# ml-rust/splintr

Measured on AMD Instinct MI355X. Metric: encode_batch MB/s (bytes in), higher is better.
Workload: dtype u8

## Files before the change

### splintr_amd/csrc/spl_common.h

```cpp
#pragma once
#include <stdint.h>

#if defined(__HIPCC__)
#include <hip/hip_runtime.h>
#define SPL_HD __host__ __device__ __forceinline__
#else
#define SPL_HD inline
#endif

namespace spl {

enum : uint32_t {
    C_P = 0,
    C_AP = 1,
    C_SP = 2,
    C_WS = 3,
    C_NL = 4,
    C_N = 5,
    C_LU = 6, C_LL = 7, C_LT = 8, C_LM = 9, C_LO = 10,
    C_M = 11,
    C_EOT = 12,
    C_WEND = 13,
    C_CONT = 15
};
#define SPL_BIT(c) (1u << (c))
constexpr uint32_t M_L = SPL_BIT(C_LU) | SPL_BIT(C_LL) | SPL_BIT(C_LT) | SPL_BIT(C_LM) | SPL_BIT(C_LO);
constexpr uint32_t M_S = SPL_BIT(C_SP) | SPL_BIT(C_WS) | SPL_BIT(C_NL);
constexpr uint32_t M_OTHER = SPL_BIT(C_P) | SPL_BIT(C_AP) | SPL_BIT(C_M);
constexpr uint32_t M_X = SPL_BIT(C_P) | SPL_BIT(C_AP) | SPL_BIT(C_SP) | SPL_BIT(C_WS) | SPL_BIT(C_M);
constexpr uint32_t M_U = SPL_BIT(C_LU) | SPL_BIT(C_LT) | SPL_BIT(C_LM) | SPL_BIT(C_LO) | SPL_BIT(C_M);
constexpr uint32_t M_W = SPL_BIT(C_LL) | SPL_BIT(C_LM) | SPL_BIT(C_LO) | SPL_BIT(C_M);
constexpr uint32_t M_UW = SPL_BIT(C_LM) | SPL_BIT(C_LO) | SPL_BIT(C_M);

constexpr uint32_t CB_CLASS = 0x0F, CB_SYNC = 0x10, CB_TSTART = 0x20, CB_LEN_SHIFT = 6;

enum : int { PAT_CL100K = 0, PAT_O200K = 1, PAT_MISTRAL_V3 = 2 };

struct alignas(16) Quad { uint32_t x, y, z, w; };
struct ShortEnt {
    uint32_t k0, k1, k2;
    uint32_t id_len;
};
constexpr int SPL_SHORT_BUCKET = 4;
constexpr int SPL_TINY_WORDS = 2;
constexpr int SPL_TINY_MAX = 4;
constexpr int SPL_T8_WORDS = 3;
constexpr int SPL_T8_MAX = 8;
constexpr int SPL_TINY_SALT_BITS = 16, SPL_T8_SALT_BITS = 10, SPL_F4_MASK_BITS = 6;
struct LongEnt {
    uint32_t tag;
    uint32_t id;
    uint32_t off;
    uint32_t len;
};
constexpr uint32_t SPL_EMPTY = 0xFFFFFFFFu;
constexpr int SPL_SHORT_MAX = 12;
constexpr uint64_t SPL_PAIR_EMPTY = ~0ull;
constexpr int SPL_PAIR_BUCKET = 4;
constexpr uint32_t SPL_ID_BITS = 21;
constexpr uint32_t SPL_ID_MASK = (1u << SPL_ID_BITS) - 1;
constexpr uint32_t SPL_NO_RANK = 0xFFFFFFFFu;
constexpr uint32_t SPL_OVF_BIT = 1u << 23;

struct P8Bucket { uint32_t a, b; };
struct alignas(8) PfxEnt { uint32_t lm, id2; };

struct alignas(64) MemoEnt {
    uint32_t key[8];
    uint32_t meta0;
    uint32_t meta1;
    uint32_t ids[6];
};
static_assert(sizeof(MemoEnt) == 64, "one cache line");
struct alignas(64) MemoExt {
    uint32_t ids[8];
    uint32_t ends[2];
    uint32_t pad[6];
};
static_assert(sizeof(MemoExt) == 64, "one cache line");
struct alignas(32) MemoHi { uint32_t k[8]; };
constexpr int SPL_MEMO_MAX_LEN = 32, SPL_MEMO_MAX_LEN2 = 64, SPL_MEMO_TOK1 = 6, SPL_MEMO_MAX_TOK = 14;
constexpr uint32_t SPL_MEMO_LOG_WORDS = 12;
constexpr uint32_t SPL_MEMO_LOG_WORDS2 = 20;
constexpr uint32_t SPL_MEMO_LOG_REGIONS = 64;

struct DeviceTables {
    const uint16_t* ucls_stage1;
    const uint8_t* ucls_stage2;
    uint32_t ucls_shift;
    uint32_t cjk_fast;
    const ShortEnt* short_tab; uint32_t short_mask;
    const uint32_t* tiny_tab;  uint32_t tiny_mask;
    const uint32_t* t8_tab;    uint32_t t8_mask;
    const LongEnt* long_tab;   uint32_t long_mask;
    const uint8_t* key_blob;
    const uint64_t* pair_tab;  uint32_t pair_mask;
    const uint32_t* byte_id;
    uint32_t max_key_len;
    uint32_t pattern;
    uint32_t all_bytes;
    uint32_t id_limit;
    const P8Bucket* p8_tab;    uint32_t p8_mask;
    const uint16_t* len_mask;  uint32_t tiny_free, t8_free;
    uint32_t ascii_base;
    const uint32_t* akind;
    const PfxEnt* pfx;
    const uint16_t* filt4;    uint32_t filt4_shift;
    const MemoEnt* memo;      uint32_t memo_mask;
    const MemoExt* memo_ext;
    const MemoEnt* memo2;     uint32_t memo2_mask;
    const MemoExt* memo2_ext; const MemoHi* memo2_hi;
};
SPL_HD uint32_t hash_f4(uint32_t w0) { return w0 * 0x9E3779B1u; }

SPL_HD uint32_t mix32(uint32_t h) {
    h ^= h >> 16; h *= 0x7feb352du; h ^= h >> 15; h *= 0x846ca68bu; h ^= h >> 16;
    return h;
}
SPL_HD uint32_t hash_t8(uint32_t k0, uint32_t k1, uint32_t len, uint32_t salt = 0) {
    return mix32(k0 * 0x9E3779B1u ^ (k1 * 0x85EBCA77u + 0x165667B1u) ^ (len * 0x27D4EB2Fu) ^ (salt * 0xC2B2AE3Du));
}
SPL_HD uint32_t hash_tiny(uint32_t k0, uint32_t len, uint32_t salt = 0) { return hash_t8(k0, 0u, len, salt); }
SPL_HD uint32_t hash_p8(uint32_t k0, uint32_t k1) { return hash_t8(k0, k1, 9u); }
SPL_HD uint32_t p8_tag(uint32_t k0, uint32_t k1) {
    return mix32(k0 * 0x85EBCA77u ^ (k1 * 0xC2B2AE3Du + 0x27D4EB2Fu)) % 0xFFFFFEu + 1u;
}
SPL_HD uint32_t p8_match(uint32_t e0, uint32_t e1, uint32_t tag) {
    const uint32_t t0 = e0 >> 8, t1 = e1 >> 8;
    uint32_t l = 0;
    if (e0 != 0 && (t0 == tag || t0 == 0xFFFFFFu)) l = e0 & 0xFFu;
    if (e1 != 0 && (t1 == tag || t1 == 0xFFFFFFu) && (e1 & 0xFFu) > l) l = e1 & 0xFFu;
    return l;
}
SPL_HD uint32_t hash_short(uint32_t k0, uint32_t k1, uint32_t k2, uint32_t len, uint32_t salt = 0) {
    uint32_t h = k0 * 0x9E3779B1u ^ (k1 * 0x85EBCA77u + 0x165667B1u) ^ (k2 * 0xC2B2AE3Du) ^ (len * 0x27D4EB2Fu) ^ (salt * 0x165667B1u);
    return mix32(h);
}
SPL_HD uint32_t hash_long_step(uint32_t h, uint32_t w) { h = (h ^ w) * 0x9E3779B1u; return (h << 13) | (h >> 19); }
SPL_HD uint32_t hash_long_fin(uint32_t h, uint32_t len) { return mix32(h ^ len); }
SPL_HD uint32_t hash_long_tag(uint32_t h) { return mix32(h * 0x85EBCA77u + 0x3C6EF372u); }
template <int KW> SPL_HD uint32_t hash_memo_w(const uint32_t (&k)[KW], uint32_t n) {
    uint32_t h = n * 0x27D4EB2Fu + 0x165667B1u;
    for (int i = 0; i < KW; i++) { h = (h ^ k[i]) * 0x9E3779B1u; h = (h << 13) | (h >> 19); }
    return mix32(h);
}
SPL_HD uint32_t hash_memo(const uint32_t (&k)[8], uint32_t n) { return hash_memo_w<8>(k, n); }
SPL_HD uint32_t memo_slot2(uint32_t h, uint32_t mask) { const uint32_t g = ((h >> 17) | (h << 15)) * 0x85EBCA77u; return ((g ^ (g >> 15)) & mask) ^ 1u; }
SPL_HD uint32_t hash_pair(uint32_t l, uint32_t r) { return mix32(l * 0x9E3779B1u + r * 0x85EBCA77u + 0x27D4EB2Fu); }
SPL_HD uint64_t pair_key(uint32_t l, uint32_t r) { return (uint64_t)l | ((uint64_t)r << SPL_ID_BITS); }
constexpr uint64_t SPL_PAIR_KEY_MASK = (1ull << (2 * SPL_ID_BITS)) - 1;

}
```

### splintr_amd/csrc/spl_k_memo.h

```cpp
#pragma once

namespace spl {


__device__ __forceinline__ uint32_t memo_meta0(uint32_t n, uint32_t t) { return 0x80000000u | (t << 8) | n; }
constexpr uint32_t MEMO_SEEDED = 0x40000000u;
constexpr uint32_t MEMO_SEED_KEEP_IDS = 32768u;

constexpr uint32_t MISS_KNOWN = 0x80000000u;
#define MISS_N(item) (((item) >> 16) & 0x7FFFu)

#ifndef SPL_MEMO_SKIP_C
#define SPL_MEMO_SKIP_C 1
#endif
template <bool LONG, class TX, class Emit>
__device__ __forceinline__ int memo_probe(const DeviceTables& T, const TX& tx, int p, int n, Emit emit) {
    constexpr int KW = LONG ? 16 : 8;
    uint32_t k[KW];
#pragma unroll
    for (int i = 0; i < KW; i++) k[i] = 4 * i < n ? mask_tail(tx.load32(p + 4 * i), n - 4 * i) : 0u;
    const uint32_t h = hash_memo_w<KW>(k, (uint32_t)n);
    const MemoEnt* const tab = LONG ? T.memo2 : T.memo;
    const MemoExt* const ext = LONG ? T.memo2_ext : T.memo_ext;
    const uint32_t mask = LONG ? T.memo2_mask : T.memo_mask;
    const uint32_t nf = (uint32_t)(LONG ? n - SPL_MEMO_MAX_LEN : n);
    uint32_t slot = h & mask;
#pragma nounroll
    for (int way = 0; way < 2; way++) {
        const Quad* q = reinterpret_cast<const Quad*>(tab + slot);
        const Quad a = q[0], c = (SPL_MEMO_SKIP_C && n <= 16) ? Quad{0u, 0u, 0u, 0u} : q[1], m = q[2], d = q[3];
        bool eq = (a.x == k[0]) & (a.y == k[1]) & (a.z == k[2]) & (a.w == k[3]) & (c.x == k[4]) & (c.y == k[5]) & (c.z == k[6]) & (c.w == k[7]) &
                  ((m.x & 0x8000003Fu) == (0x80000000u | nf));
        if (LONG && eq) {
            const Quad* hq = reinterpret_cast<const Quad*>(T.memo2_hi + slot);
            const Quad h0 = hq[0], h1 = hq[1];
            eq = (h0.x == k[KW - 8]) & (h0.y == k[KW - 7]) & (h0.z == k[KW - 6]) & (h0.w == k[KW - 5]) &
                 (h1.x == k[KW - 4]) & (h1.y == k[KW - 3]) & (h1.z == k[KW - 2]) & (h1.w == k[KW - 1]);
        }
        if (eq) {
            const uint32_t nt = (m.x >> 8) & 15u;
            if (nt == 0u) return 2;
            const uint32_t ids[6] = {m.z, m.w, d.x, d.y, d.z, d.w};
            int at = 0;
#pragma unroll
            for (int t = 0; t < SPL_MEMO_TOK1; t++)
                if ((uint32_t)t < nt) { emit(p + at, ids[t]); if (t < 5) at = (int)((m.y >> (6 * t)) & 63u); }
            if (nt > (uint32_t)SPL_MEMO_TOK1) {
                const Quad* x = reinterpret_cast<const Quad*>(ext + slot);
                const Quad e0 = x[0], e1 = x[1], e2 = x[2];
                const uint32_t xi[8] = {e0.x, e0.y, e0.z, e0.w, e1.x, e1.y, e1.z, e1.w};
#pragma unroll
                for (int t = 0; t < 8; t++)
                    if ((uint32_t)(t + SPL_MEMO_TOK1) < nt) {
                        at = (int)(((t < 5 ? e2.x : e2.y) >> (6 * (t % 5))) & 63u);
                        emit(p + at, xi[t]);
                    }
            }
            return 1;
        }
        if (!(m.x >> 31)) return 0;
        slot = memo_slot2(h, mask);
    }
    return 0;
}

template <bool LONG, class TX>
__device__ __forceinline__ void memo_log_part(const Batch& b, const TX& tx, const uint32_t* list, uint32_t m16, uint32_t c16, uint32_t m64, uint32_t tile) {
    constexpr int KW = LONG ? 16 : 8;
    constexpr uint32_t LW = LONG ? SPL_MEMO_LOG_WORDS2 : SPL_MEMO_LOG_WORDS;
    const uint32_t lane = tidx() & 63u;
    auto eligible = [&](uint32_t item) {
        const uint32_t n = MISS_N(item);
        return !(item & MISS_KNOWN) && (LONG ? n > (uint32_t)SPL_MEMO_MAX_LEN && n <= (uint32_t)SPL_MEMO_MAX_LEN2 : n <= (uint32_t)SPL_MEMO_MAX_LEN);
    };
    uint32_t n_el = 0;
    if (!LONG) for (uint32_t i0 = 0; i0 < m16; i0 += 64u) n_el += (uint32_t)__popcll(__ballot(i0 + lane < m16 && eligible(list[i0 + lane])));
    for (uint32_t i0 = 0; i0 < m64; i0 += 64u) n_el += (uint32_t)__popcll(__ballot(i0 + lane < m64 && eligible(list[c16 + i0 + lane])));
    if (!n_el) return;
    const uint32_t cap = LONG ? b.mlog2_cap : b.mlog_cap;
    const uint32_t region = tile % SPL_MEMO_LOG_REGIONS;
    uint32_t base = 0;
    if (lane == 0u) base = atomicAdd(&b.mlog_cnt[(LONG ? SPL_MEMO_LOG_REGIONS : 0) + region], n_el);
    base = (uint32_t)__builtin_amdgcn_readfirstlane((int)base);
    if (base >= cap) return;
    const uint32_t ask = cap / 2u < 512u ? cap / 2u : 512u;
    if (lane == 0u && base < ask && base + n_el >= ask) *b.mflag = 1u;
    uint32_t* const out = (LONG ? b.mlog2 : b.mlog) + ((size_t)region * cap) * LW;
    auto put = [&](uint32_t slot, uint32_t item) {
        if (base + slot >= cap) return;
        const int p = (int)(item & 0xFFFFu), n = (int)MISS_N(item);
        uint32_t* e = out + (size_t)(base + slot) * LW;
        e[0] = (uint32_t)n;
#pragma unroll
        for (int i = 0; i < KW; i++) e[1 + i] = 4 * i < n ? mask_tail(tx.load32(p + 4 * i), n - 4 * i) : 0u;
    };
    uint32_t slot = 0;
    for (int part = LONG ? 1 : 0; part < 2; part++) {
        const uint32_t cnt = part ? m64 : m16, at = part ? c16 : 0u;
        for (uint32_t i0 = 0; i0 < cnt; i0 += 64u) {
            const uint32_t i = i0 + lane;
            const uint32_t item = i < cnt ? list[at + i] : MISS_KNOWN;
            const bool el = i < cnt && eligible(item);
            const unsigned long long em = __ballot(el);
            if (el) put(slot + mbcnt64(em), item);
            slot += (uint32_t)__popcll(em);
        }
    }
}
template <class TX>
__device__ __forceinline__ void memo_log(const Batch& b, const TX& tx, const uint32_t* list, uint32_t m16, uint32_t c16, uint32_t m64, uint32_t tile) {
    memo_log_part<false>(b, tx, list, m16, c16, m64, tile);
    if (b.mlog2 && m64) memo_log_part<true>(b, tx, list, m16, c16, m64, tile);
}

constexpr int MEMO_FILL_NT = 128, MEMO_FILL_NT2 = 64;
template <int NT_> struct MemoNodes {
    uint32_t* id_; uint32_t* rk_;
    __device__ __forceinline__ uint32_t& id(int i) { return id_[i * NT_]; }
    __device__ __forceinline__ uint32_t& rk(int i) { return rk_[i * NT_]; }
};
struct MemoKeyAcc {
    const uint32_t* k;
    __device__ __forceinline__ uint32_t txt(int q) const { return (k[q >> 2] >> (8 * (q & 3))) & 0xFFu; }
};
template <bool LONG>
__global__ __launch_bounds__(LONG ? MEMO_FILL_NT2 : MEMO_FILL_NT) void k_memo_fill(DeviceTables T, MemoEnt* memo, MemoExt* memo_ext, MemoHi* memo_hi, const uint32_t* mlog,
                                                                               const uint32_t* mlog_cnt, uint32_t mlog_cap, uint32_t* claim, uint32_t round, unsigned long long* stats) {
    constexpr int KW = LONG ? 16 : 8, NTF = LONG ? MEMO_FILL_NT2 : MEMO_FILL_NT, NMAX = LONG ? SPL_MEMO_MAX_LEN2 : SPL_MEMO_MAX_LEN;
    constexpr uint32_t LW = LONG ? SPL_MEMO_LOG_WORDS2 : SPL_MEMO_LOG_WORDS;
    const uint32_t region = blockIdx.y, i = blockIdx.x * blockDim.x + threadIdx.x;
    const uint32_t cnt = mlog_cnt[region] < mlog_cap ? mlog_cnt[region] : mlog_cap;
    if (i >= cnt) return;
    const uint32_t* e = mlog + ((size_t)region * mlog_cap + i) * LW;
    const uint32_t n = e[0];
    uint32_t k[KW];
#pragma unroll
    for (int w = 0; w < KW; w++) k[w] = e[1 + w];
    if (n < (LONG ? (uint32_t)SPL_MEMO_MAX_LEN + 1u : 2u) || n > (uint32_t)NMAX) return;
    const uint32_t mask = LONG ? T.memo2_mask : T.memo_mask;
    const uint32_t nf = LONG ? n - (uint32_t)SPL_MEMO_MAX_LEN : n;
    const uint32_t h = hash_memo_w<KW>(k, n);
    const uint32_t slots[2] = {h & mask, memo_slot2(h, mask)};
    auto holds = [&](uint32_t sl) {
        const MemoEnt* me = memo + sl;
        bool same = (me->meta0 & 0x8000003Fu) == (0x80000000u | nf);
#pragma unroll
        for (int w = 0; w < 8; w++) same = same && me->key[w] == k[w];
        if (LONG) {
#pragma unroll
            for (int w = 0; w < 8; w++) same = same && memo_hi[sl].k[w] == k[KW - 8 + w];
        }
        return same;
    };
    const bool taken0 = (memo[slots[0]].meta0 >> 31) != 0u, taken1 = (memo[slots[1]].meta0 >> 31) != 0u;
    if ((taken0 && holds(slots[0])) || (taken0 && taken1 && holds(slots[1]))) return;
    MemoEnt* me = nullptr;
    if (!taken0) { if (atomicExch(&claim[slots[0]], round) != round) me = memo + slots[0]; }
    if (!me && taken0 && !taken1) { if (atomicExch(&claim[slots[1]], round) != round) me = memo + slots[1]; }
    if (!me && taken0 && taken1) {
        const bool spare_seed = (!(round & 1u) || memo[slots[0]].ids[0] < MEMO_SEED_KEEP_IDS) && (memo[slots[0]].meta0 & MEMO_SEEDED) && !(memo[slots[1]].meta0 & MEMO_SEEDED);
        const uint32_t ev = slots[spare_seed ? 1 : 0];
        if (atomicExch(&claim[ev], round) != round) me = memo + ev;
    }
    if (!me) return;
    __shared__ uint32_t s_id[NMAX * NTF], s_rk[NMAX * NTF];
    MemoNodes<NTF> s{s_id + threadIdx.x, s_rk + threadIdx.x};
    const MemoKeyAcc tx{k};
    bpe_serial(T, s, tx, 0, (int)n);
    uint32_t ids[SPL_MEMO_MAX_TOK], ends = 0, ends2[2] = {0u, 0u}, nt = 0;
#pragma unroll
    for (int t = 0; t < SPL_MEMO_MAX_TOK; t++) ids[t] = 0u;
    bool fits = true;
    for (uint32_t q = 0; q < n; q++) {
        const uint32_t id = s.id((int)q);
        if (id == SPL_DEAD) continue;
        if (nt >= 1u && nt <= 5u) ends |= q << (6u * (nt - 1u));
        else if (nt >= 6u && nt <= 13u) ends2[(nt - 6u) / 5u] |= q << (6u * ((nt - 6u) % 5u));
        if (id >= T.id_limit || nt >= (uint32_t)SPL_MEMO_MAX_TOK) { fits = false; break; }
        ids[nt++] = id;
    }
    me->meta0 = 0u;
#pragma unroll
    for (int w = 0; w < 8; w++) me->key[w] = k[w];
    if (LONG) {
        MemoHi* const mh = memo_hi + (me - memo);
// ... 38 lines not shown
```

### splintr_amd/csrc/spl_k_merge.h

```cpp
#pragma once

namespace spl {

struct LdsAcc {
    const uint8_t* rec_;
    const uint8_t* txt_;
    __device__ __forceinline__ uint32_t rec(int q) const { return rec_[q]; }
    __device__ __forceinline__ uint32_t txt(int q) const { return txt_[q]; }
    __device__ __forceinline__ uint32_t load32(int p) const {
        const uint32_t* w = reinterpret_cast<const uint32_t*>(txt_) + (p >> 2);
        return __builtin_amdgcn_alignbyte(w[1], w[0], p & 3);
    }
};

extern "C" __device__ int spl_writelane(int src, int lane, int old) __asm("llvm.amdgcn.writelane.i32");
#define write_lane(v, s, lane_) spl_writelane((int)(s), (lane_), (v))

struct WaveBV {
    uint32_t x;
    __device__ __forceinline__ WaveBV operator&(const WaveBV& o) const { return WaveBV{x & o.x}; }
    __device__ __forceinline__ WaveBV operator|(const WaveBV& o) const { return WaveBV{x | o.x}; }
    __device__ __forceinline__ WaveBV operator~() const { return WaveBV{~x}; }
    __device__ __forceinline__ WaveBV shl1() const {
        const uint32_t prev = (uint32_t)__builtin_amdgcn_update_dpp(0, (int)x, 0x138, 0xF, 0xF, true);
        return WaveBV{(x << 1) | (prev >> 31)};
    }
    __device__ __forceinline__ WaveBV shr1() const {
        const uint32_t next = (uint32_t)__builtin_amdgcn_update_dpp(0, (int)x, 0x130, 0xF, 0xF, true);
        return WaveBV{(x >> 1) | (next << 31)};
    }
    __device__ __forceinline__ bool any() const { return __any(x != 0u); }
};

struct MaskLdsAcc {
    const uint8_t* rec_;
    const uint8_t* txt_;
    const uint32_t* mk_;
    int nbw_, w_;
    bool eot_;
    __device__ __forceinline__ uint32_t rec(int q) const { return rec_[q]; }
    __device__ __forceinline__ uint32_t txt(int q) const { return txt_[q]; }
    __device__ __forceinline__ uint32_t mw(int which, int w) const { return mk_[which * nbw_ + w]; }
    __device__ __forceinline__ int wbits() const { return w_; }
    __device__ __forceinline__ bool end_is_eot() const { return eot_; }
};

constexpr int LONG_SMALL_NMAX = 128;
__device__ __forceinline__ void push_long(const Batch& b, uint32_t pos, uint32_t len) {
    if (len <= (uint32_t)LONG_SMALL_NMAX) {
        const uint32_t i = atomicAdd(&b.qcount[2], 1u);
        if (i < b.qcaplong) b.qlong[i] = make_uint2(pos, len);
    } else {
        const uint32_t i = atomicAdd(&b.qcount[4], 1u);
        if (i < b.qcaplong) b.qlong[b.qcaplong - 1u - i] = make_uint2(pos, len);
    }
}

__device__ __forceinline__ uint32_t row16_min(uint32_t x) {
#ifndef SPL_NO_DPP_ASM
    asm volatile("s_nop 1\n\tv_min_u32_dpp %0, %0, %0 quad_perm:[1,0,3,2] row_mask:0xf bank_mask:0xf\n\t"
                 "s_nop 1\n\tv_min_u32_dpp %0, %0, %0 quad_perm:[2,3,0,1] row_mask:0xf bank_mask:0xf\n\t"
                 "s_nop 1\n\tv_min_u32_dpp %0, %0, %0 row_half_mirror row_mask:0xf bank_mask:0xf\n\t"
                 "s_nop 1\n\tv_min_u32_dpp %0, %0, %0 row_mirror row_mask:0xf bank_mask:0xf"
                 : "+v"(x));
    return x;
#else
    auto step = [](uint32_t v, uint32_t y) { return y < v ? y : v; };
    x = step(x, (uint32_t)__builtin_amdgcn_update_dpp((int)x, (int)x, 0xB1, 0xF, 0xF, false));
    x = step(x, (uint32_t)__builtin_amdgcn_update_dpp((int)x, (int)x, 0x4E, 0xF, 0xF, false));
    x = step(x, (uint32_t)__builtin_amdgcn_update_dpp((int)x, (int)x, 0x141, 0xF, 0xF, false));
    x = step(x, (uint32_t)__builtin_amdgcn_update_dpp((int)x, (int)x, 0x140, 0xF, 0xF, false));
    return x;
#endif
}
#ifndef SPL_PAIR_SHORT
#define SPL_PAIR_SHORT 1
#endif
__device__ __forceinline__ uint32_t row_min_sub(uint32_t x, bool whole_row) {
    asm volatile("s_nop 1\n\tv_min_u32_dpp %0, %0, %0 quad_perm:[1,0,3,2] row_mask:0xf bank_mask:0xf\n\t"
                 "s_nop 1\n\tv_min_u32_dpp %0, %0, %0 quad_perm:[2,3,0,1] row_mask:0xf bank_mask:0xf\n\t"
                 "s_nop 1\n\tv_min_u32_dpp %0, %0, %0 row_half_mirror row_mask:0xf bank_mask:0xf"
                 : "+v"(x));
    uint32_t y = x;
    asm volatile("s_nop 1\n\tv_min_u32_dpp %0, %0, %0 row_mirror row_mask:0xf bank_mask:0xf" : "+v"(y));
    return whole_row ? y : x;
}
template <int GW> __device__ __forceinline__ uint32_t group_min(uint32_t x, int sub = GW) {
    if (GW == 16 && SPL_PAIR_SHORT) return row_min_sub(x, sub == 16);
    x = row16_min(x);
    if (GW == 32) {
#ifndef SPL_NO_PERMLANE_SWAP
        const auto r = __builtin_amdgcn_permlane16_swap(x, x, false, false);
        const uint32_t a = r[0], c = r[1];
        x = a < c ? a : c;
#else
        const uint32_t y = (uint32_t)__builtin_amdgcn_ds_swizzle((int)x, 0x401F);
        x = y < x ? y : x;
#endif
    }
    return x;
}

__device__ __forceinline__ uint32_t wave_scan_incl(uint32_t x) {
    x += (uint32_t)__builtin_amdgcn_update_dpp(0, (int)x, 0x111, 0xF, 0xF, true);
    x += (uint32_t)__builtin_amdgcn_update_dpp(0, (int)x, 0x112, 0xF, 0xF, true);
    x += (uint32_t)__builtin_amdgcn_update_dpp(0, (int)x, 0x114, 0xF, 0xF, true);
    x += (uint32_t)__builtin_amdgcn_update_dpp(0, (int)x, 0x118, 0xF, 0xF, true);
    x += (uint32_t)__builtin_amdgcn_update_dpp(0, (int)x, 0x142, 0xA, 0xF, false);
    x += (uint32_t)__builtin_amdgcn_update_dpp(0, (int)x, 0x143, 0xC, 0xF, false);
    return x;
}

__device__ __forceinline__ uint32_t wave_scan_max(uint32_t x) {
    auto mx = [](uint32_t a, int b) { return a > (uint32_t)b ? a : (uint32_t)b; };
    x = mx(x, __builtin_amdgcn_update_dpp(0, (int)x, 0x111, 0xF, 0xF, true));
    x = mx(x, __builtin_amdgcn_update_dpp(0, (int)x, 0x112, 0xF, 0xF, true));
    x = mx(x, __builtin_amdgcn_update_dpp(0, (int)x, 0x114, 0xF, 0xF, true));
    x = mx(x, __builtin_amdgcn_update_dpp(0, (int)x, 0x118, 0xF, 0xF, true));
    x = mx(x, __builtin_amdgcn_update_dpp(0, (int)x, 0x142, 0xA, 0xF, false));
    x = mx(x, __builtin_amdgcn_update_dpp(0, (int)x, 0x143, 0xC, 0xF, false));
    return x;
}

__device__ __forceinline__ uint32_t nib_transpose8(uint32_t v) {
    const uint32_t l = tidx() & 7u;
    {
        uint32_t t = (uint32_t)__builtin_amdgcn_update_dpp((int)v, (int)v, 0x104, 0xF, 0x5, false);
        t = (uint32_t)__builtin_amdgcn_update_dpp((int)t, (int)v, 0x114, 0xF, 0xA, false);
        const uint32_t km = (l & 4u) ? 0xFFFF0000u : 0x0000FFFFu;
        const uint32_t y = __builtin_amdgcn_alignbit(t, t, 16);
        v = (v & km) | (y & ~km);
    }
    {
        const uint32_t t = (uint32_t)__builtin_amdgcn_update_dpp((int)v, (int)v, 0x4E, 0xF, 0xF, false);
        const uint32_t km = (l & 2u) ? 0xFF00FF00u : 0x00FF00FFu;
        const uint32_t y = __builtin_amdgcn_alignbit(t, t, (l & 2u) ? 8u : 24u);
        v = (v & km) | (y & ~km);
    }
    {
        const uint32_t t = (uint32_t)__builtin_amdgcn_update_dpp((int)v, (int)v, 0xB1, 0xF, 0xF, false);
        const uint32_t km = (l & 1u) ? 0xF0F0F0F0u : 0x0F0F0F0Fu;
        const uint32_t y = __builtin_amdgcn_alignbit(t, t, (l & 1u) ? 4u : 28u);
        v = (v & km) | (y & ~km);
    }
    return v;
}

template <int NW> __device__ __forceinline__ int next_set_bit(const uint32_t (&a)[NW], int from) {
    int res = -1;
#pragma unroll
    for (int w = NW - 1; w >= 0; w--) {
        uint32_t x = a[w];
        const int lo = from - 32 * w;
        if (lo >= 32) x = 0;
        else if (lo > 0) x &= ~((1u << lo) - 1u);
        if (x) res = 32 * w + __ffs((int)x) - 1;
    }
    return res;
}
template <int NW> __device__ __forceinline__ int prev_set_bit(const uint32_t (&a)[NW], int before) {
    int res = -1;
#pragma unroll
    for (int w = 0; w < NW; w++) {
        uint32_t x = a[w];
        const int hi = before - 32 * w;
// ... 1024 lines not shown
```

### splintr_amd/csrc/spl_k_pretok.h

```cpp
#pragma once

namespace spl {

#ifndef SPL_XCD_MAP
#define SPL_XCD_MAP 1
#endif
__device__ __forceinline__ uint32_t xcd_tile() {
    if (!SPL_XCD_MAP) return blockIdx.x;
    const uint32_t x = blockIdx.x & 7u, j = blockIdx.x >> 3, q = gridDim.x >> 3, r = gridDim.x & 7u;
    return x * q + (x < r ? x : r) + j;
}
constexpr uint32_t PRETOK_E_TSTART = 1u, PRETOK_E_SKIP = 2u, PRETOK_E_GAPS = 4u, PRETOK_E_EXT = 8u, PRETOK_E_FUSE = 64u, PRETOK_E_MEMO1 = 128u;
inline uint32_t pretok_flags(const DeviceTables& T, const Batch& b) {
    return (b.tstart ? PRETOK_E_TSTART : 0u) | (b.skip ? PRETOK_E_SKIP : 0u) | (b.ext_gaps ? PRETOK_E_GAPS : 0u) |
           (b.ext_starts ? PRETOK_E_EXT : 0u) | (T.pattern << 4) | (b.ftc ? PRETOK_E_FUSE : 0u) | ((b.memo_first && T.memo) ? PRETOK_E_MEMO1 : 0u) |
           (b.tile0 << 8);
}
struct PretokKernargs {
    const uint8_t* e_text; const uint64_t* e_doc_off; uint32_t e_n_bytes, e_n_docs; unsigned long long* e_dbg;
    const uint32_t* e_akind; uint32_t e_flags; DeviceTables T; Batch b;
};
#define PRETOK_EARLY(T, b) (b).text, (b).doc_off, (b).n_bytes, (b).n_docs, (b).dbg, (T).akind, pretok_flags(T, b)
template <int TB_, int RH_>
__global__ __launch_bounds__(NT) __attribute__((amdgpu_waves_per_eu(SPL_PRETOK_WAVES)))
// ... 338 lines not shown
                } else if (KPAT != PAT_CL100K) {
                    const bool mistral = KPAT == PAT_MISTRAL_V3;
                    const O200kStartMasks<WaveBV> om{WaveBV{ld(MK_L)}, WaveBV{ld(MK_UP)}, WaveBV{ld(MK_LB)}, WaveBV{ld(MK_N)}, WaveBV{ld(MK_S)},
                                                     WaveBV{ld(MK_NL)}, WaveBV{ld(MK_O)}, WaveBV{ld(MK_AP)}, WaveBV{ld(MK_SP)},
                                                     WaveBV{ld(MK_SL)}, WaveBV{ld(MK_CS)}, WaveBV{ts}};
                    bool ok = true;
                    uint32_t bits;
                    if (part == 0) bits = o200k_starts_ln(om, mistral, ok, 16).x | range_word(fe, fe + 1);
                    else if (part == 2) bits = o200k_starts_s(om, mistral, ok, 16).x;
                    else {
                        WaveBV CAND;
                        bits = o200k_starts_o(om, mistral, CAND, ok, 16).x;
                        uint32_t ca = mistral ? 0u : CAND.x & own;
                        const LdsAcc acc{s_rec, s_txt};
                        bool chain = false;
                        while (ca) {
                            const int ap = ln * 32 + __ffs((int)ca) - 1;
                            ca &= ca - 1;
                            int e;
                            if (!o200k_contraction_at(acc, ap, e)) chain = true;
                            else if (e > 0) {
                                for (int q = ap; q < e; q++) atomicOr(&s_kill[q >> 5], 1u << (q & 31));
                                if (e < fe) atomicOr(&s_add[e >> 5], 1u << (e & 31));
                            }
                        }
                        if (__any(chain)) ok = false;
                    }
                    bits &= range_word(fs, fe + 1);
                    if (ok) {
                        fine = 1;
                        if (bits) atomicOr(&s_cbits[ln], bits);
                    }
                } else {
                    const Cl100kStartMasks<WaveBV> cm{WaveBV{ld(MK_L)}, WaveBV{ld(MK_N)}, WaveBV{ld(MK_S)}, WaveBV{ld(MK_NL)},
                                                      WaveBV{ld(MK_O)}, WaveBV{ld(MK_AP)}, WaveBV{ld(MK_SP)}, WaveBV{ld(MK_CS)}, WaveBV{ts}};
                    bool ok = true;
                    uint32_t bits;
                    if (part == 0) bits = cl100k_starts_ln(cm, ok, 16).x | ts | range_word(fe, fe + 1);
                    else if (part == 2) bits = cl100k_starts_s(cm, ok, 16).x;
                    else {
                        WaveBV CA;
                        bits = cl100k_starts_o(cm, CA).x;
                        uint32_t ca = CA.x & own;
                        const LdsAcc acc{s_rec, s_txt};
                        while (ca) {
                            const int ap = ln * 32 + __ffs((int)ca) - 1;
                            ca &= ca - 1;
                            const int e = contraction(acc, ap);
                            if (e > 0 && e < fe) atomicOr(&s_cbits[e >> 5], 1u << (e & 31));
                        }
                    }
                    bits &= range_word(fs, fe + 1);
                    if (ok) {
                        fine = 1;
                        if (bits) atomicOr(&s_cbits[ln], bits);
                    }
                }
            }
        }
        if (ln == 0 && fine) atomicAdd(&s_fast, 1u);
    }
    }
    if (SPL_MASK_STARTS && DIRECT) __syncthreads();
    const bool fast_starts = SPL_MASK_STARTS && DIRECT && s_fast == 3u;
    SPL_STAMP(3);

    {
        uint32_t word = 0;
        if (fast_starts) {
            if (tid < G::NBW) word = (s_cbits[tid] & ~s_kill[tid]) | s_add[tid];
        } else if (tid < G::NBW) {
            word = s_mk[MK_SY * NBW1 + tid];
            const int lo = LH - tid * 32, hi = LH + TB_ - tid * 32;
            if (hi <= 0 || lo >= 32) word = 0;
            else {
                if (lo > 0) word &= ~0u << lo;
                if (hi < 32) word &= (1u << hi) - 1u;
            }
        }
        static_assert(G::NBW <= 64, "the window's bitmap words must fit one wavefront");
        if (tid < 64) {
            const uint32_t cnt = __popc(word);
            const uint32_t x = wave_scan_incl(cnt);
            uint32_t base = x - cnt;
            if (tid == 63) s_total = x;
            while (word) {
                const int bit = __ffs(word) - 1;
                word &= word - 1;
                s_cpos[base++] = (uint16_t)(tid * 32 + bit);
            }
        }
        __syncthreads();
    }
    {
        const MaskLdsAcc acc{s_rec, s_txt, s_mk, NBW1, Wv, (B - w0) <= (int64_t)Wv};
        const int nsync = fast_starts ? 0 : (int)s_total;
        auto push_defer = [&](uint32_t gpos) {
            if (DIRECT && !b.qcount) {
                const uint32_t qi = atomicAdd(&s_dq[1], 1u);
                if (qi < 2) s_dq[2 + qi] = gpos;
            } else {
                const uint32_t qi = atomicAdd(&b.qcount[3], 1u);
                if (qi < b.qcapdefer) b.qdefer[qi] = gpos;
            }
        };
        for (int k = tid; k < nsync; k += NT) {
            int p = s_cpos[k];
            for (;;) {
                const int e = match_end_m(acc, p, KPAT);
                if (e == SPL_DEFER) {
                    push_defer((uint32_t)(w0 + p));
                    break;
                }
                s_chunk[atomicAdd(&s_nch, 1u)] = (uint32_t)p | ((uint32_t)(e - p) << 16);
                p = e;
                if (p >= Wv) {
                    if (w0 + p < B) push_defer((uint32_t)(w0 + p) | 0x80000000u);
                    break;
                }
                if (((s_mk[MK_SY * NBW1 + (p >> 5)] | s_mk[MK_TS * NBW1 + (p >> 5)]) >> (p & 31)) & 1u) break;
            }
        }
        if (!fast_starts) __syncthreads();
    }
    SPL_STAMP(4);

    SPL_STAMP(5);

    {
        LdsAcc tx{s_rec, s_txt};
        const bool from_list = LIST_CHUNKS && !fast_starts;
        const int K = from_list ? (int)s_nch + 1 : (int)s_total;
        const bool memo_first = (e_flags & PRETOK_E_MEMO1) != 0u;
        for (int k = tid; k + 1 < K; k += NT) {
            int p, n;
            if (from_list) {
                const uint32_t c = s_chunk[k];
                p = (int)(c & 0xFFFFu); n = (int)(c >> 16);
            } else {
                p = s_cpos[k];
                if (ext ? ((s_sk[p >> 5] >> (p & 31)) & 1u) != 0u : (s_rec[p] & CB_CLASS) >= C_EOT) continue;
                n = (int)s_cpos[k + 1] - p;
            }
            auto memo_put = [&](int q, uint32_t tid_) { s_ids[q] = tid_; atomicOr(&s_tbits[q >> 5], 1u << (q & 31)); };
            const bool m_short = T.memo && n > 1 && n <= SPL_MEMO_MAX_LEN && p + n <= Wv;
            const bool m_long = T.memo2 && n > SPL_MEMO_MAX_LEN && n <= SPL_MEMO_MAX_LEN2 && p + n <= Wv;
            uint32_t id = SPL_NO_RANK;
            int held = 0;
            if (memo_first) {
                if (n == 1) {
                    id = T.byte_id[s_txt[p]];
                    if (id >= T.id_limit) id = SPL_NO_RANK;
                } else {
                    if (m_short) held = memo_probe<false>(T, tx, p, n, memo_put);
                    else if (m_long) held = memo_probe<true>(T, tx, p, n, memo_put);
                    if (held == 0) id = probe_chunk_tile(T, tx, p, n);
                }
            } else {
                id = probe_chunk_tile(T, tx, p, n);
                if (id == SPL_NO_RANK && n > 1) {
                    held = m_short ? memo_probe<false>(T, tx, p, n, memo_put) : 0;
                    if (m_long) held = memo_probe<true>(T, tx, p, n, memo_put);
                }
            }
#ifdef SPL_MEMO_STATS
            if (e_dbg && id == SPL_NO_RANK && n > 1) atomicAdd(&e_dbg[4 + ((m_short || m_long) ? 1 + held : 0)], 1ull);
#endif
            if (id != SPL_NO_RANK) {
                if (DIRECT) s_ids[p] = id;
                else b.stage[w0 + p] = id;
                atomicOr(&s_tbits[p >> 5], 1u << (p & 31));
            } else if (n > 1 && held != 1) {
                const uint32_t item = (uint32_t)p | ((uint32_t)n << 16) | (held == 2 ? MISS_KNOWN : 0u);
                if (TILE_LIST) {
                    if (n <= 64 || !b.qcount) s_tmiss[atomicAdd(&s_nq[0], 1u)] = item;
                    else push_long(b, (uint32_t)(w0 + p), (uint32_t)n);
                }
                else if (n <= 16) s_miss[atomicAdd(&s_nq[0], 1u)] = item;
                else if (n <= 64) {
                    bool sent = false;
                    if (DIRECT && !b.qcount && ((s_txt[p] | s_txt[p + 1]) & 0x80u)) {
                        const uint32_t m = atomicAdd(&s_dq[11], 1u);
                        if (m < (uint32_t)DIRECT_LQ_MEDIUM) {
                            s_lq[2 * (DIRECT_LQCAP - 1 - m)] = (uint32_t)(w0 + p);
                            s_lq[2 * (DIRECT_LQCAP - 1 - m) + 1] = (uint32_t)n;
                            sent = true;
                        }
                    }
                    if (!sent) s_miss[G::C16 + atomicAdd(&s_nq[1], 1u)] = item;
                } else if (DIRECT && !b.qcount) {
                    const uint32_t qi = atomicAdd(&s_dq[0], 1u);
                    s_lq[2 * qi] = (uint32_t)(w0 + p);
                    s_lq[2 * qi + 1] = (uint32_t)n;
                } else push_long(b, (uint32_t)(w0 + p), (uint32_t)n);
            }
        }
    }
    __syncthreads();
    SPL_STAMP(6);

    if (DIRECT) __builtin_amdgcn_s_setprio(SPL_MERGE_PRIO);
#ifndef SPL_MERGE_SKIP
#define SPL_MERGE_SKIP 1
#endif
    const uint32_t m16 = TILE_LIST ? 0u : (uint32_t)__builtin_amdgcn_readfirstlane((int)s_nq[0]);
    const uint32_t m64 = TILE_LIST ? 0u : (uint32_t)__builtin_amdgcn_readfirstlane((int)s_nq[1]);
    const bool do_short = !SPL_MERGE_SKIP || m16 != 0u, do_medium = !SPL_MERGE_SKIP || m64 != 0u;
    if (!TILE_LIST) {
#ifndef SPL_SORT_SHORT
#define SPL_SORT_SHORT 1
#endif
        constexpr bool SORT_SHORT = SPL_SORT_SHORT && Wv <= 1024;
        if (SORT_SHORT && do_short) {
            uint32_t my_item[(G::C16 + NT - 1) / NT], my_r[(G::C16 + NT - 1) / NT];
#pragma unroll
            for (int q = 0; q < (G::C16 + NT - 1) / NT; q++) {
                const uint32_t k = tid + q * NT;
                if (k < m16) { my_item[q] = s_miss[k]; my_r[q] = atomicAdd(&s_scnt[16 - MISS_N(my_item[q])], 1u); }
            }
            __syncthreads();
            if (tid < 64) {
                const uint32_t c = tid < 17 ? s_scnt[tid] : 0u;
                const uint32_t x = wave_scan_incl(c);
                if (tid < 17) s_scnt[tid] = x - c;
            }
            __syncthreads();
#pragma unroll
            for (int q = 0; q < (G::C16 + NT - 1) / NT; q++) {
                const uint32_t k = tid + q * NT;
                if (k < m16) {
                    const uint32_t n = MISS_N(my_item[q]);
                    s_cpos[s_scnt[16 - n] + my_r[q]] = (uint16_t)((my_item[q] & 0x3FFu) | ((n - 1) << 10));
                }
            }
            __syncthreads();
        }
        uint32_t* const stage_w0 = b.stage + w0;
        auto put = [&](int q, uint32_t id) {
            if (id >= T.id_limit) return;
            if (DIRECT && q >= Wv) {
                const uint32_t g = (uint32_t)(w0 + q);
                __hip_atomic_store(&b.stage[g], id, __ATOMIC_RELAXED, __HIP_MEMORY_SCOPE_AGENT);
                atomicOr(&b.tbits[g >> 5], 1u << (g & 31));
                atomicMax(&s_dq[4], g + 1u);
                return;
            }
            if (DIRECT) s_ids[q] = id;
            else stage_w0[q] = id;
            atomicOr(&s_tbits[q >> 5], 1u << (q & 31));
        };
        const int lane = tid & 63;
#ifdef SPL_DEBUG_STAMPS
        const long long ws_t0 = clock64();
        uint32_t ws_nmed = 0, ws_nshort = 0;
        long long ws_wt[6] = {0, 0, 0, 0, 0, 0};
#endif
        if (do_medium) for (;;) {
            uint32_t it = 0;
            if (lane == 0) it = atomicAdd(&s_nq[3], SPL_MEDIUM_PAIRS ? 2u : 1u);
            it = __builtin_amdgcn_readfirstlane(it);
            if (it >= m64) break;
#ifdef SPL_SKIP_MEDIUM
            continue;
#endif
#ifdef SPL_DEBUG_STAMPS
            ws_nmed++;
#endif
            if (DIRECT && SPL_MEDIUM_PRIO != SPL_MERGE_PRIO) __builtin_amdgcn_s_setprio(SPL_MEDIUM_PRIO);
            const uint32_t itemA = s_miss[G::C16 + it];
            const uint32_t itemB = (SPL_MEDIUM_PAIRS && it + 1u < m64) ? s_miss[G::C16 + it + 1u] : 0u;
            const int pA = (int)(itemA & 0xFFFFu), nA = (int)MISS_N(itemA), pB = (int)(itemB & 0xFFFFu), nB = (int)MISS_N(itemB);
            bool pair = SPL_MEDIUM_PAIRS && nA <= 32 && nB <= 32;
            if (pair) {
                const int half = lane >> 5, hl = lane & 31;
                const int p = half ? pB : pA, n = half ? nB : nA;
                if (__any(hl < n && (s_txt[p + hl] & 0x80u))) pair = false;
                else {
#if defined(SPL_DEBUG_STAMPS) && defined(SPL_STAMP_MEDIUM)
                    long long* const wtm = (e_dbg && blockIdx.x == SPL_DBG_WG && ws_nmed == 1) ? ws_wt : nullptr;
#else
                    long long* const wtm = nullptr;
#endif
                    bpe_group_tab<32>(T, LdsAcc{s_rec, s_txt}, p, n, s_sub[(tid >> 6) * 4 + half * 2],
                                      [&](int i, uint32_t id) {
                                          put(p + i, id);
                                      }, wtm);
                }
            }
            if (!pair) {
                bpe_wave64_tab(T, LdsAcc{s_rec, s_txt}, pA, nA, s_sub[(tid >> 6) * 4],
                               [&](int i, uint32_t id) {
                                   put(pA + i, id);
                               });
                if (nB) bpe_wave64_tab(T, LdsAcc{s_rec, s_txt}, pB, nB, s_sub[(tid >> 6) * 4],
                                       [&](int i, uint32_t id) {
                                           put(pB + i, id);
                                       });
            }
        }
        if (DIRECT && SPL_MEDIUM_PRIO != SPL_MERGE_PRIO) __builtin_amdgcn_s_setprio(SPL_MERGE_PRIO);
        SPL_STAMP(9);
#ifdef SPL_DEBUG_STAMPS
        const long long ws_t1 = clock64();
#endif
        const uint32_t first8 = (SPL_PAIR_SHORT && SORT_SHORT) ? s_scnt[8] : m16;
        const uint32_t nslots = first8 + (m16 - first8 + 1u) / 2u;
        if (do_short) for (;;) {
            uint32_t it = 0;
            if ((lane & 15) == 0) it = atomicAdd(&s_nq[2], 1u);
            it = __shfl(it, lane & ~15);
            const bool slot = it < nslots;
            if (!__any(slot)) break;
#ifdef SPL_SKIP_SHORT
            continue;
#endif
// ... 543 lines not shown
```

### splintr_amd/csrc/spl_lookup.h

```cpp
#pragma once
#include "spl_common.h"

namespace spl {

constexpr uint32_t SPL_DEAD = 0xFFFFFFFEu;

SPL_HD uint32_t mask_tail(uint32_t w, int nbytes) {
    return nbytes >= 4 ? w : nbytes <= 0 ? 0u : (w & ((1u << (8 * nbytes)) - 1u));
}

SPL_HD bool bucket_overflowed(uint32_t last) { return last != SPL_EMPTY && (last & SPL_OVF_BIT) != 0u; }

SPL_HD uint32_t key_salt(const DeviceTables& T, uint32_t k0) { return (uint32_t)T.len_mask[k0 & 0xFFFFu] >> 8; }
SPL_HD uint32_t tiny_salt(const DeviceTables& T, uint32_t k0) { return T.pfx[k0 & 0xFFFFu].lm >> 16; }
SPL_HD uint32_t t8_salt(const DeviceTables& T, uint32_t k0) { return (uint32_t)T.filt4[hash_f4(k0) >> T.filt4_shift] >> SPL_F4_MASK_BITS; }

SPL_HD uint32_t probe_tiny(const DeviceTables& T, uint32_t k0, uint32_t n, uint32_t salt) {
    const uint32_t* e = T.tiny_tab + (size_t)(hash_tiny(k0, n, salt) & T.tiny_mask) * SPL_TINY_WORDS;
    const uint32_t ek = e[0], ei = e[1];
    return ((ek == k0) & ((ei >> 24) == n)) ? (ei & SPL_ID_MASK) : SPL_NO_RANK;
}
SPL_HD uint32_t probe_t8(const DeviceTables& T, uint32_t k0, uint32_t k1, uint32_t n, uint32_t salt) {
    const uint32_t* e = T.t8_tab + (size_t)(hash_t8(k0, k1, n, salt) & T.t8_mask) * SPL_T8_WORDS;
    const uint32_t e0 = e[0], e1 = e[1], ei = e[2];
    return ((e0 == k0) & (e1 == k1) & ((ei >> 24) == n)) ? (ei & SPL_ID_MASK) : SPL_NO_RANK;
}
SPL_HD uint32_t probe_short12(const DeviceTables& T, uint32_t k0, uint32_t k1, uint32_t k2, uint32_t n, uint32_t salt) {
    uint32_t bkt = hash_short(k0, k1, k2, n, salt) & T.short_mask;
    for (;;) {
        const Quad* q = reinterpret_cast<const Quad*>(T.short_tab + (size_t)bkt * SPL_SHORT_BUCKET);
        const Quad e0 = q[0], e1 = q[1], e2 = q[2], e3 = q[3];
        const bool f0 = (e0.x == k0) & (e0.y == k1) & (e0.z == k2) & ((e0.w >> 24) == n);
        const bool f1 = (e1.x == k0) & (e1.y == k1) & (e1.z == k2) & ((e1.w >> 24) == n);
        const bool f2 = (e2.x == k0) & (e2.y == k1) & (e2.z == k2) & ((e2.w >> 24) == n);
        const bool f3 = (e3.x == k0) & (e3.y == k1) & (e3.z == k2) & ((e3.w >> 24) == n);
        uint32_t r = SPL_NO_RANK;
        r = f3 ? (e3.w & SPL_ID_MASK) : r;
        r = f2 ? (e2.w & SPL_ID_MASK) : r;
        r = f1 ? (e1.w & SPL_ID_MASK) : r;
        r = f0 ? (e0.w & SPL_ID_MASK) : r;
        if ((f0 | f1 | f2 | f3) | !bucket_overflowed(e3.w)) return r;
        bkt = (bkt + 1) & T.short_mask;
    }
}
SPL_HD uint32_t probe_short(const DeviceTables& T, uint32_t k0, uint32_t k1, uint32_t k2, uint32_t n) {
    if (n <= (uint32_t)SPL_TINY_MAX) return probe_tiny(T, k0, n, tiny_salt(T, k0));
    if (n <= (uint32_t)SPL_T8_MAX) return probe_t8(T, k0, k1, n, t8_salt(T, k0));
    return probe_short12(T, k0, k1, k2, n, key_salt(T, k0));
}

template <class TX> SPL_HD uint32_t probe_long(const DeviceTables& T, const TX& tx, int p, int n) {
    uint32_t h = 0;
    for (int i = 0; i < n; i += 4) h = hash_long_step(h, mask_tail(tx.load32(p + i), n - i));
    h = hash_long_fin(h, (uint32_t)n);
    const uint32_t tag = hash_long_tag(h);
    uint32_t slot = h & T.long_mask;
    for (;;) {
        const LongEnt e = T.long_tab[slot];
        if (e.id == SPL_EMPTY) return SPL_NO_RANK;
        if (e.tag == tag && e.len == (uint32_t)n) {
            const uint32_t* kw = reinterpret_cast<const uint32_t*>(T.key_blob + e.off);
            bool eq = true;
            for (int i = 0; i < n && eq; i += 4) eq = kw[i >> 2] == mask_tail(tx.load32(p + i), n - i);
            if (eq) return e.id;
        }
        slot = (slot + 1) & T.long_mask;
    }
}

template <class TX> SPL_HD uint32_t probe_chunk(const DeviceTables& T, const TX& tx, int p, int n) {
    if (n <= SPL_SHORT_MAX) {
        const uint32_t k0 = mask_tail(tx.load32(p), n);
        const uint32_t k1 = n > 4 ? mask_tail(tx.load32(p + 4), n - 4) : 0u;
        const uint32_t k2 = n > 8 ? mask_tail(tx.load32(p + 8), n - 8) : 0u;
        return probe_short(T, k0, k1, k2, (uint32_t)n);
    }
    if ((uint32_t)n > T.max_key_len) return SPL_NO_RANK;
    return probe_long(T, tx, p, n);
}

SPL_HD uint32_t pair_rank(const DeviceTables& T, uint32_t l, uint32_t r) {
    if ((l | r) > SPL_ID_MASK) return SPL_NO_RANK;
    const uint64_t key = pair_key(l, r);
    const uint32_t klo = (uint32_t)key, khi = (uint32_t)(key >> 32);
    uint32_t bkt = hash_pair(l, r) & T.pair_mask;
    for (;;) {
        const Quad* q = reinterpret_cast<const Quad*>(T.pair_tab + (size_t)bkt * SPL_PAIR_BUCKET);
        const Quad a = q[0], c = q[1];
        const bool f0 = (a.x == klo) & ((a.y & 0x3FFu) == khi);
        const bool f1 = (a.z == klo) & ((a.w & 0x3FFu) == khi);
        const bool f2 = (c.x == klo) & ((c.y & 0x3FFu) == khi);
        const bool f3 = (c.z == klo) & ((c.w & 0x3FFu) == khi);
        uint32_t res = SPL_NO_RANK;
        res = f3 ? (c.w >> 10) : res;
        res = f2 ? (c.y >> 10) : res;
        res = f1 ? (a.w >> 10) : res;
        res = f0 ? (a.y >> 10) : res;
        if ((f0 | f1 | f2 | f3) | ((c.z & c.w) == 0xFFFFFFFFu)) return res;
        bkt = (bkt + 1) & T.pair_mask;
    }
}

struct PairProbe { Quad a, c; uint32_t bkt, klo, khi; bool valid; };
SPL_HD void pair_issue(const DeviceTables& T, uint32_t l, uint32_t r, PairProbe& pp) {
    pp.valid = (l | r) <= SPL_ID_MASK;
    const uint64_t key = pair_key(l & SPL_ID_MASK, r & SPL_ID_MASK);
    pp.klo = (uint32_t)key; pp.khi = (uint32_t)(key >> 32);
    pp.bkt = hash_pair(l & SPL_ID_MASK, r & SPL_ID_MASK) & T.pair_mask;
    const Quad* q = reinterpret_cast<const Quad*>(T.pair_tab + (size_t)pp.bkt * SPL_PAIR_BUCKET);
    pp.a = q[0]; pp.c = q[1];
}
SPL_HD uint32_t pair_finish(const DeviceTables& T, const PairProbe& pp) {
    if (!pp.valid) return SPL_NO_RANK;
    const bool f0 = (pp.a.x == pp.klo) & ((pp.a.y & 0x3FFu) == pp.khi);
    const bool f1 = (pp.a.z == pp.klo) & ((pp.a.w & 0x3FFu) == pp.khi);
    const bool f2 = (pp.c.x == pp.klo) & ((pp.c.y & 0x3FFu) == pp.khi);
    const bool f3 = (pp.c.z == pp.klo) & ((pp.c.w & 0x3FFu) == pp.khi);
    uint32_t res = SPL_NO_RANK;
    res = f3 ? (pp.c.w >> 10) : res;
    res = f2 ? (pp.c.y >> 10) : res;
    res = f1 ? (pp.a.w >> 10) : res;
    res = f0 ? (pp.a.y >> 10) : res;
    if ((f0 | f1 | f2 | f3) | ((pp.c.z & pp.c.w) == 0xFFFFFFFFu)) return res;
    uint32_t bkt = (pp.bkt + 1) & T.pair_mask;
    for (;;) {
        const Quad* q = reinterpret_cast<const Quad*>(T.pair_tab + (size_t)bkt * SPL_PAIR_BUCKET);
        const Quad a = q[0], c = q[1];
        const bool g0 = (a.x == pp.klo) & ((a.y & 0x3FFu) == pp.khi);
        const bool g1 = (a.z == pp.klo) & ((a.w & 0x3FFu) == pp.khi);
        const bool g2 = (c.x == pp.klo) & ((c.y & 0x3FFu) == pp.khi);
        const bool g3 = (c.z == pp.klo) & ((c.w & 0x3FFu) == pp.khi);
        uint32_t r2 = SPL_NO_RANK;
        r2 = g3 ? (c.w >> 10) : r2;
        r2 = g2 ? (c.y >> 10) : r2;
        r2 = g1 ? (a.w >> 10) : r2;
        r2 = g0 ? (a.y >> 10) : r2;
        if ((g0 | g1 | g2 | g3) | ((c.z & c.w) == 0xFFFFFFFFu)) return r2;
        bkt = (bkt + 1) & T.pair_mask;
    }
}

template <class S, class TX> SPL_HD void bpe_serial(const DeviceTables& T, S& s, const TX& tx, int p, int n) {
    for (int i0 = 0; i0 < n; i0 += 8) {
        uint32_t bb[8], iv[8];
#pragma unroll
        for (int k = 0; k < 8; k++) bb[k] = i0 + k < n ? tx.txt(p + i0 + k) : 0u;
#pragma unroll
        for (int k = 0; k < 8; k++) iv[k] = T.byte_id[bb[k]];
#pragma unroll
        for (int k = 0; k < 8; k++) if (i0 + k < n) s.id(i0 + k) = iv[k];
    }
    for (int i0 = 0; i0 + 1 < n; i0 += 4) {
        PairProbe pp[4];
#pragma unroll
        for (int k = 0; k < 4; k++) {
            const bool on = i0 + k + 1 < n;
            pair_issue(T, on ? s.id(i0 + k) : 0u, on ? s.id(i0 + k + 1) : 0u, pp[k]);
        }
#pragma unroll
        for (int k = 0; k < 4; k++) if (i0 + k + 1 < n) s.rk(i0 + k) = pair_finish(T, pp[k]);
    }
// ... 31 lines not shown
```

Before: 55310.

## Flatten memo hash and size key loads to wave-uniform word count

Replaces the serial multiply-rotate memo hash with independent per-word terms XORed together, which shortens the dependency chain. Key words are now built from aligned LDS loads combined with alignbyte, and the number of words loaded and hashed is chosen per wave (2, 4 or 8) based on the longest chunk in the wave. The second key quad is skipped when the wave's chunks are short. The hash function changes, so host-built memo tables must use the same hash, and the word-count branch adds wave-level votes.

Result: no change. 55760, median of 6 (+0.8%).

```diff
diff --git a/splintr_amd/csrc/spl_common.h b/splintr_amd/csrc/spl_common.h
--- a/splintr_amd/csrc/spl_common.h
+++ b/splintr_amd/csrc/spl_common.h
@@ -139,11 +139,32 @@
 SPL_HD uint32_t hash_long_step(uint32_t h, uint32_t w) { h = (h ^ w) * 0x9E3779B1u; return (h << 13) | (h >> 19); }
 SPL_HD uint32_t hash_long_fin(uint32_t h, uint32_t len) { return mix32(h ^ len); }
 SPL_HD uint32_t hash_long_tag(uint32_t h) { return mix32(h * 0x85EBCA77u + 0x3C6EF372u); }
-template <int KW> SPL_HD uint32_t hash_memo_w(const uint32_t (&k)[KW], uint32_t n) {
+#ifndef SPL_MEMO_HASH_FLAT
+#define SPL_MEMO_HASH_FLAT 1
+#endif
+SPL_HD uint32_t hash_memo_term(uint32_t w, int i) {
+    const uint32_t x = w * (0x9E3779B1u + 0x3C6EF372u * (uint32_t)i);
+    const int r = (7 * i + 5) % 31 + 1;
+#if defined(__clang__)
+    return __builtin_rotateleft32(x, (uint32_t)r);
+#else
+    return (x << r) | (x >> (32 - r));
+#endif
+}
+template <int KW> SPL_HD uint32_t hash_memo_nw(const uint32_t (&k)[KW], uint32_t n, int nw) {
     uint32_t h = n * 0x27D4EB2Fu + 0x165667B1u;
+#if SPL_MEMO_HASH_FLAT
+#if defined(__HIPCC__)
+#pragma unroll
+#endif
+    for (int i = 0; i < KW; i++) if (i < nw) h ^= hash_memo_term(k[i], i);
+#else
+    (void)nw;
     for (int i = 0; i < KW; i++) { h = (h ^ k[i]) * 0x9E3779B1u; h = (h << 13) | (h >> 19); }
+#endif
     return mix32(h);
 }
+template <int KW> SPL_HD uint32_t hash_memo_w(const uint32_t (&k)[KW], uint32_t n) { return hash_memo_nw<KW>(k, n, KW); }
 SPL_HD uint32_t hash_memo(const uint32_t (&k)[8], uint32_t n) { return hash_memo_w<8>(k, n); }
 SPL_HD uint32_t memo_slot2(uint32_t h, uint32_t mask) { const uint32_t g = ((h >> 17) | (h << 15)) * 0x85EBCA77u; return ((g ^ (g >> 15)) & mask) ^ 1u; }
 SPL_HD uint32_t hash_pair(uint32_t l, uint32_t r) { return mix32(l * 0x9E3779B1u + r * 0x85EBCA77u + 0x27D4EB2Fu); }
diff --git a/splintr_amd/csrc/spl_k_memo.h b/splintr_amd/csrc/spl_k_memo.h
--- a/splintr_amd/csrc/spl_k_memo.h
+++ b/splintr_amd/csrc/spl_k_memo.h
@@ -13,13 +13,33 @@
 #ifndef SPL_MEMO_SKIP_C
 #define SPL_MEMO_SKIP_C 1
 #endif
+#ifndef SPL_MEMO_KEY_ROUND
+#define SPL_MEMO_KEY_ROUND 1
+#endif
 template <bool LONG, class TX, class Emit>
-__device__ __forceinline__ int memo_probe(const DeviceTables& T, const TX& tx, int p, int n, Emit emit) {
+__device__ __forceinline__ int memo_probe(const DeviceTables& T, const TX& tx, int p, int n, int wlast, Emit emit) {
     constexpr int KW = LONG ? 16 : 8;
     uint32_t k[KW];
+    uint32_t h;
+    bool wide = true;
+#if SPL_MEMO_KEY_ROUND
+#pragma unroll
+    for (int i = 0; i < KW; i++) k[i] = 0u;
+    if (LONG) {
+        memo_key_words<16>(tx, p, n, wlast, k); h = hash_memo_nw<KW>(k, (uint32_t)n, 16);
+    } else if (!__any(n > 8)) {
+        memo_key_words<2>(tx, p, n, wlast, k); h = hash_memo_nw<KW>(k, (uint32_t)n, 2); wide = false;
+    } else if (!__any(n > 16)) {
+        memo_key_words<4>(tx, p, n, wlast, k); h = hash_memo_nw<KW>(k, (uint32_t)n, 4); wide = false;
+    } else {
+        memo_key_words<8>(tx, p, n, wlast, k); h = hash_memo_nw<KW>(k, (uint32_t)n, 8);
+    }
+#else
+    (void)wlast;
 #pragma unroll
     for (int i = 0; i < KW; i++) k[i] = 4 * i < n ? mask_tail(tx.load32(p + 4 * i), n - 4 * i) : 0u;
-    const uint32_t h = hash_memo_w<KW>(k, (uint32_t)n);
+    h = hash_memo_w<KW>(k, (uint32_t)n);
+#endif
     const MemoEnt* const tab = LONG ? T.memo2 : T.memo;
     const MemoExt* const ext = LONG ? T.memo2_ext : T.memo_ext;
     const uint32_t mask = LONG ? T.memo2_mask : T.memo_mask;
@@ -28,9 +48,9 @@
 #pragma nounroll
     for (int way = 0; way < 2; way++) {
         const Quad* q = reinterpret_cast<const Quad*>(tab + slot);
-        const Quad a = q[0], c = (SPL_MEMO_SKIP_C && n <= 16) ? Quad{0u, 0u, 0u, 0u} : q[1], m = q[2], d = q[3];
-        bool eq = (a.x == k[0]) & (a.y == k[1]) & (a.z == k[2]) & (a.w == k[3]) & (c.x == k[4]) & (c.y == k[5]) & (c.z == k[6]) & (c.w == k[7]) &
-                  ((m.x & 0x8000003Fu) == (0x80000000u | nf));
+        const Quad a = q[0], c = (!wide || (SPL_MEMO_SKIP_C && n <= 16)) ? Quad{0u, 0u, 0u, 0u} : q[1], m = q[2], d = q[3];
+        bool eq = (a.x == k[0]) & (a.y == k[1]) & (a.z == k[2]) & (a.w == k[3]) & ((m.x & 0x8000003Fu) == (0x80000000u | nf));
+        if (wide) eq = eq & (c.x == k[4]) & (c.y == k[5]) & (c.z == k[6]) & (c.w == k[7]);
         if (LONG && eq) {
             const Quad* hq = reinterpret_cast<const Quad*>(T.memo2_hi + slot);
             const Quad h0 = hq[0], h1 = hq[1];
diff --git a/splintr_amd/csrc/spl_k_merge.h b/splintr_amd/csrc/spl_k_merge.h
--- a/splintr_amd/csrc/spl_k_merge.h
+++ b/splintr_amd/csrc/spl_k_merge.h
@@ -11,6 +11,7 @@
         const uint32_t* w = reinterpret_cast<const uint32_t*>(txt_) + (p >> 2);
         return __builtin_amdgcn_alignbyte(w[1], w[0], p & 3);
     }
+    __device__ __forceinline__ uint32_t aligned32(int w) const { return reinterpret_cast<const uint32_t*>(txt_)[w]; }
 };
 
 extern "C" __device__ int spl_writelane(int src, int lane, int old) __asm("llvm.amdgcn.writelane.i32");
diff --git a/splintr_amd/csrc/spl_k_pretok.h b/splintr_amd/csrc/spl_k_pretok.h
--- a/splintr_amd/csrc/spl_k_pretok.h
+++ b/splintr_amd/csrc/spl_k_pretok.h
@@ -514,15 +514,15 @@
                     id = T.byte_id[s_txt[p]];
                     if (id >= T.id_limit) id = SPL_NO_RANK;
                 } else {
-                    if (m_short) held = memo_probe<false>(T, tx, p, n, memo_put);
-                    else if (m_long) held = memo_probe<true>(T, tx, p, n, memo_put);
+                    if (m_short) held = memo_probe<false>(T, tx, p, n, G::NW32 - 1, memo_put);
+                    else if (m_long) held = memo_probe<true>(T, tx, p, n, G::NW32 - 1, memo_put);
                     if (held == 0) id = probe_chunk_tile(T, tx, p, n);
                 }
             } else {
                 id = probe_chunk_tile(T, tx, p, n);
                 if (id == SPL_NO_RANK && n > 1) {
-                    held = m_short ? memo_probe<false>(T, tx, p, n, memo_put) : 0;
-                    if (m_long) held = memo_probe<true>(T, tx, p, n, memo_put);
+                    held = m_short ? memo_probe<false>(T, tx, p, n, G::NW32 - 1, memo_put) : 0;
+                    if (m_long) held = memo_probe<true>(T, tx, p, n, G::NW32 - 1, memo_put);
                 }
             }
 #ifdef SPL_MEMO_STATS
diff --git a/splintr_amd/csrc/spl_lookup.h b/splintr_amd/csrc/spl_lookup.h
--- a/splintr_amd/csrc/spl_lookup.h
+++ b/splintr_amd/csrc/spl_lookup.h
@@ -7,6 +7,29 @@
 
 SPL_HD uint32_t mask_tail(uint32_t w, int nbytes) {
     return nbytes >= 4 ? w : nbytes <= 0 ? 0u : (w & ((1u << (8 * nbytes)) - 1u));
+}
+
+SPL_HD uint32_t align_bytes(uint32_t hi, uint32_t lo, uint32_t s) {
+#if defined(__HIP_DEVICE_COMPILE__)
+    return __builtin_amdgcn_alignbyte(hi, lo, s);
+#else
+    return (uint32_t)((((uint64_t)hi << 32) | lo) >> (8u * s));
+#endif
+}
+
+template <int NW, class TX>
+SPL_HD void memo_key_words(const TX& tx, int p, int n, int wlast, uint32_t* k) {
+    const int w0 = p >> 2;
+    const uint32_t s = (uint32_t)p & 3u;
+    uint32_t w[NW + 1];
+#if defined(__HIPCC__)
+#pragma unroll
+#endif
+    for (int i = 0; i <= NW; i++) w[i] = tx.aligned32(i <= 4 ? w0 + i : (w0 + i < wlast ? w0 + i : wlast));
+#if defined(__HIPCC__)
+#pragma unroll
+#endif
+    for (int i = 0; i < NW; i++) k[i] = mask_tail(align_bytes(w[i + 1], w[i], s), n - 4 * i);
 }
 
 SPL_HD bool bucket_overflowed(uint32_t last) { return last != SPL_EMPTY && (last & SPL_OVF_BIT) != 0u; }
```
